# apache/auron

Measured on AMD Instinct MI355X. Metric: tpcds_suite_seconds, lower is better.
Workload: dtype decimal64/fp64

## Files before the change

auron_amd/config.py:

```python
from __future__ import annotations

import os
from dataclasses import dataclass
from typing import Any, Dict, Optional


@dataclass(frozen=True)
class ConfigOption:
    key: str
    default: Any
    typ: type
    doc: str = ""
    env: Optional[str] = None


_REGISTRY: Dict[str, ConfigOption] = {}


def _opt(key: str, default, typ, doc="", env=None) -> ConfigOption:
    o = ConfigOption(key, default, typ, doc, env)
    _REGISTRY[key] = o
    return o


# ... 55 lines not shown
                                    "below this many rows partial-agg "
                                    "skipping is never sampled")
SORT_LIMIT_TOPK = _opt("spark.auron.sort.topK.enable", True, bool,
                       "ORDER BY+LIMIT keeps only the top K rows per batch")
SORT_EXTERNAL_WIDE_KEYS = _opt("spark.auron.sort.external.wideKeys.enable",
                               True, bool,
                               "range-split external sort also for string and "
                               "decimal128 first keys (off: such sorts stay "
                               "monolithic and cannot spill)",
                               env="AURON_SORT_EXTERNAL_WIDE_KEYS")
EXCHANGE_SAMPLE_ROWS = _opt("spark.auron.rangePartition.sampleRows", 4096, int,
                            "per-rank sample size for range-partition bounds")
SCAN_CACHE_BYTES = _opt("spark.auron.scan.cache.maxBytes", 0, int,
                        "per-query decoded-scan cache budget; 0 = auto "
                        "(15% of HBM on GPU, 4 GB on CPU)",
                        env="AURON_SCAN_CACHE_BYTES")
STREAM_BYTES = _opt("spark.auron.stream.minInputBytes", -1, int,
                    "estimated agg-input bytes above which operators "
                    "stream instead of materializing; -1 = auto (8% of "
                    "HBM on GPU, 1 GB on CPU), 0 = always stream",
                    env="AURON_STREAM_BYTES")
SCAN_HBM_CACHE = _opt("spark.auron.scan.hbmStagedCache.maxBytes", 0, int,
                      "staged raw-page bytes kept device-resident across "
                      "reads; 0 = auto (30% of HBM)",
                      env="AURON_SCAN_HBM_CACHE")
HBM_CACHE_RESERVE = _opt("spark.auron.scan.hbmStagedCache.reserveFraction",
                         0.25, float,
                         "free-HBM fraction the staged-bytes cache must "
                         "never consume (evicts itself under pressure)")
SCAN_DELTA_NATIVE = _opt("spark.auron.scan.deltaNative.enable", True, bool,
                         "decode DELTA_BINARY_PACKED pages and "
                         "DELTA_LENGTH_BYTE_ARRAY / DELTA_BYTE_ARRAY string "
                         "pages with the k_pq_delta_* kernels from a "
                         "host-built miniblock index, DELTA_BYTE_ARRAY "
                         "strings rebuilt by k_pq_dba_bytes (off: "
                         "DELTA_BINARY_PACKED is expanded to PLAIN by one "
                         "host job per page and DELTA_LENGTH_BYTE_ARRAY and "
                         "DELTA_BYTE_ARRAY columns take the pyarrow host "
                         "read)",
                         env="AURON_SCAN_DELTA_NATIVE")
SCAN_PREFETCH = _opt("spark.auron.scan.streamPrefetch", 2, int,
                     "files decoded ahead of the consumer on the "
                     "streaming scan path")
SCAN_IO_THREADS = _opt("spark.auron.scan.ioThreads", 8, int,
                       "host page-read/staging thread-pool size",
                       env="AURON_SCAN_IO_THREADS")
STREAM_PEEK_FACTOR = _opt("spark.auron.stream.peekBatches", 8, int,
                          "batch-size multiples buffered before the "
                          "chunked agg commits to streaming")
STREAM_JOIN_PROBE = _opt("spark.auron.stream.joinProbe.enable", True, bool,
                         "probe build-right joins batch-by-batch on the "
                         "streaming path (GPU only)",
                         env="AURON_STREAM_JOIN_PROBE")
SPILL_DIR = _opt("spark.auron.spill.dir", "", str,
                 "directory for disk-tier spill files (empty = system tmp)",
                 env="AURON_SPILL_DIR")
MEM_BUDGET = _opt("spark.auron.memory.budgetBytes", 0, int,
                  "absolute memmgr budget override; 0 = memoryFraction "
                  "of device/host memory", env="AURON_MEM_BUDGET")


class AuronConf:
    def __init__(self, overrides: Optional[Dict[str, Any]] = None):
        self._values: Dict[str, Any] = {}
        if overrides:
            for k, v in overrides.items():
                self.set(k, v)

    def set(self, key: str, value) -> "AuronConf":
        if key not in _REGISTRY:
            raise KeyError(f"unknown config {key}; known: {sorted(_REGISTRY)}")
        self._values[key] = value
        return self

    def get(self, opt: ConfigOption):
        if opt.key in self._values:
            return self._values[opt.key]
        if opt.env and opt.env in os.environ:
            raw = os.environ[opt.env]
            if opt.typ is bool:
                return raw not in ("0", "false", "False")
            return opt.typ(raw)
        return opt.default

    @staticmethod
    def options() -> Dict[str, ConfigOption]:
        return dict(_REGISTRY)
```

auron_amd/engine/executor.py:

```python
from __future__ import annotations

import os
import time
from dataclasses import dataclass, field
from typing import Dict, List, Optional

import torch
import torch.distributed as dist

from .. import dtypes, ops
from ..column import Column, RecordBatch, adjacent_equal, compact_validity
from ..dtypes import DataType
from ..exchange import all_gather_batch, all_to_all
from ..exprs import AggFunc, Col
from ..plan import nodes as P
from ..config import AGG_STREAMING, BROADCAST_CACHE_BYTES, AuronConf
from .window import exec_window


@dataclass
class ExecContext:
    device: torch.device = torch.device("cpu")
    rank: int = 0
    world_size: int = 1
# ... 1744 lines not shown
                left = _concat(left_batches())
            else:
                lb = _concat(left_batches())
                left = _concat(all_gather_batch(lb, self.ctx.device, self.ctx.group))
                right = _concat(self.execute(node.right))
        else:
            right = _concat(self.execute(node.right))
            left = _concat(left_batches())
        if cache_entry is not None and cache_entry.get("batch") is None:
            cache_entry["batch"] = right
            self.ctx.broadcast_cache_bytes += sum(
                c.data.numel() * c.data.element_size() for c in right.columns)
        if not node.broadcast:
            from ..config import (SMJ_FALLBACK_ENABLE, SMJ_FALLBACK_ROWS,
                                  AuronConf)

            conf = AuronConf()
            build = right if node.build_side == "right" else left
            if (conf.get(SMJ_FALLBACK_ENABLE)
                    and build.num_rows > conf.get(SMJ_FALLBACK_ROWS)
                    and node.how in ("inner", "left", "right", "full",
                                     "semi", "anti", "existence")):
                smj = P.SortMergeJoin(P.MemoryScan([left]), P.MemoryScan([right]),
                                      node.left_keys, node.right_keys,
                                      how=node.how,
                                      existence_col=node.existence_col,
                                      residual=node.residual)
                return self._exec_SortMergeJoin(smj)
        lkeys = [k.eval(left) for k in node.left_keys]
        rkeys = [k.eval(right) for k in node.right_keys]
        lkeys, rkeys = _normalize_join_keys(lkeys, rkeys)
        how = node.how
        device = self.ctx.device

        table = None
        if cache_entry is not None and node.build_side == "right":
            sig = _expr_sig(node.right_keys)
            table = cache_entry["tables"].get(sig)
            if table is None:
                table = ops.join_build(rkeys)
                if table is not None:
                    cache_entry["tables"][sig] = table
                    self.ctx.broadcast_cache_bytes += table.nbytes

        if node.residual is not None:
            bi, pi, _ = ops.hash_join(rkeys, lkeys,
                                      emit_unmatched_probe=False,
                                      need_build_matched=False,
                                      table=table)
            return self._finish_join_pairs(left, right, pi, bi, how,
                                           node.residual, node.existence_col)

        if how in ("semi", "anti", "existence"):
            counts = ops.join_counts(rkeys, lkeys)
            if how == "semi":
                return [left.filter(counts > 0)]
            if how == "anti":
                return [left.filter(counts == 0)]
            exists = Column(dtypes.bool_, counts > 0)
            return [RecordBatch(left.names + [node.existence_col], left.columns + [exists])]

        preserved = {"inner": set(), "left": {"left"}, "right": {"right"},
                     "full": {"left", "right"}}[how]
        build_side = node.build_side
        probe_side = "left" if build_side == "right" else "right"
        build_keys, probe_keys = (rkeys, lkeys) if build_side == "right" else (lkeys, rkeys)
        bi, pi, bmatched = ops.hash_join(
            build_keys, probe_keys,
            emit_unmatched_probe=(probe_side in preserved),
            need_build_matched=(build_side in preserved),
            table=table if build_side == "right" else None,
        )
        if build_side in preserved and bmatched is not None:
            un = torch.nonzero(~bmatched, as_tuple=False).flatten()
            if un.numel():
                bi = torch.cat([bi, un])
                pi = torch.cat([pi, torch.full((un.numel(),), -1, dtype=torch.int64, device=bi.device)])
        li, ri = (pi, bi) if build_side == "right" else (bi, pi)
        out_left = left.gather(li, may_have_negative=True)
        out_right = right.gather(ri, may_have_negative=True)
        return [RecordBatch(out_left.names + out_right.names,
                            out_left.columns + out_right.columns)]

    def _finish_join_pairs(self, left: RecordBatch, right: RecordBatch,
                           li: torch.Tensor, ri: torch.Tensor, how: str,
                           residual, existence_col: str) -> List[RecordBatch]:
        device = self.ctx.device
        if residual is not None and li.numel():
            pair = RecordBatch(left.names + right.names,
                               left.gather(li).columns + right.gather(ri).columns)
            m = residual.eval(pair)
            keep = m.data
            if m.validity is not None:
                keep = keep & m.validity
            li, ri = li[keep], ri[keep]
        nl, nr = left.num_rows, right.num_rows
        if how in ("semi", "anti", "existence"):
            lmatched = torch.zeros(nl, dtype=torch.bool, device=device)
            if li.numel():
                lmatched[li] = True
            if how == "semi":
                return [left.filter(lmatched)]
            if how == "anti":
                return [left.filter(~lmatched)]
            return [RecordBatch(left.names + [existence_col],
                                left.columns + [Column(dtypes.bool_, lmatched)])]
        preserved = {"inner": set(), "left": {"left"}, "right": {"right"},
                     "full": {"left", "right"}}[how]
        if "left" in preserved:
            lm = torch.zeros(nl, dtype=torch.bool, device=device)
            if li.numel():
                lm[li] = True
# ... 53 lines not shown
```

auron_amd/exchange.py:

```python
from __future__ import annotations

from typing import List, Optional, Tuple

import torch
import torch.distributed as dist

from . import dtypes
from .column import Column, RecordBatch
from .dtypes import DataType

_ALIGN = 8


def _pad8(x: int) -> int:
    return (x + _ALIGN - 1) & ~(_ALIGN - 1)


def _byte_view(t: torch.Tensor) -> torch.Tensor:
    if t.numel() == 0:
        return torch.empty(0, dtype=torch.uint8, device=t.device)
    t = t.contiguous()
    if t.dtype == torch.bool:
        t = t.view(torch.uint8)
    t = t.view(torch.uint8) if t.dtype != torch.uint8 else t
# ... 109 lines not shown
        if b is None:
            metas.append(None)
            bufs.append(torch.zeros(0, dtype=torch.uint8, device=device))
        else:
            if schema is None:
                schema = _schema_of(b)
            m, buf = pack_batch(b, device)
            metas.append(m)
            bufs.append(buf)
    if schema is not None and all(m is not None for m in metas):
        ncols = len(schema)
        stride = 1 + 3 * ncols + 1
        comm_dev = device if dist.get_backend(group) == "nccl" else "cpu"
        sz = torch.full((world, stride), -1, dtype=torch.int64)
        for d, m in enumerate(metas):
            sz[d, 0] = m["nrows"]
            for i, cm in enumerate(m["cols"]):
                sz[d, 1 + 3 * i] = cm["data"]
                sz[d, 2 + 3 * i] = cm["val"]
                sz[d, 3 + 3 * i] = cm["off"]
            sz[d, -1] = bufs[d].numel()
        sz = sz.reshape(-1).to(comm_dev)
        outs = [torch.empty_like(sz) for _ in range(world)]
        dist.all_gather(outs, sz, group=group)
        rows = [o.cpu().reshape(world, stride)[rank] for o in outs]
        recv_metas = [_meta_from_sizes(schema, r) for r in rows]
        recv_sizes = [int(r[-1]) for r in rows]
    else:
        payload = (metas, [b.numel() for b in bufs])
        gathered: List[Optional[tuple]] = [None] * world
        dist.all_gather_object(gathered, payload, group=group)
        recv_metas = [gathered[s][0][rank] for s in range(world)]
        recv_sizes = [int(gathered[s][1][rank]) for s in range(world)]

    backend = dist.get_backend(group)
    out_batches: List[RecordBatch] = []
    if backend == "nccl":
        send_flat = torch.cat(bufs) if sum(b.numel() for b in bufs) else torch.zeros(0, dtype=torch.uint8, device=device)
        recv_total = sum(recv_sizes)
        recv_flat = torch.empty(recv_total, dtype=torch.uint8, device=device)
        dist.all_to_all_single(
            recv_flat, send_flat,
            output_split_sizes=recv_sizes,
            input_split_sizes=[b.numel() for b in bufs],
            group=group,
        )
        out_batches = _split_recv_flat(recv_flat, recv_sizes, recv_metas)
    else:
        recv_bufs: List[Optional[torch.Tensor]] = [None] * world
        recv_bufs[rank] = bufs[rank]
        for other in range(world):
            if other == rank:
                continue
            rb = torch.empty(recv_sizes[other], dtype=torch.uint8, device=device)
            if rank < other:
                if bufs[other].numel():
                    dist.send(bufs[other], dst=other, group=group)
                if rb.numel():
                    dist.recv(rb, src=other, group=group)
            else:
                if rb.numel():
                    dist.recv(rb, src=other, group=group)
                if bufs[other].numel():
                    dist.send(bufs[other], dst=other, group=group)
            recv_bufs[other] = rb
        for s in range(world):
            if recv_metas[s] is not None:
                out_batches.append(unpack_batch(recv_metas[s], recv_bufs[s]))
    return out_batches


def _split_recv_flat(recv_flat: torch.Tensor, recv_sizes, recv_metas):
    out = []
    pos = 0
    for s in range(len(recv_sizes)):
        nb = recv_sizes[s]
        if recv_metas[s] is not None:
            out.append(unpack_batch(recv_metas[s], recv_flat[pos:pos + nb]))
        pos += nb
    return out


def all_gather_batch(batch: Optional[RecordBatch], device, group=None) -> List[RecordBatch]:
    world = dist.get_world_size(group)
    if batch is not None:
        meta, buf = pack_batch(batch, device)
    else:
        meta, buf = None, torch.zeros(0, dtype=torch.uint8, device=device)
    gathered: List[Optional[tuple]] = [None] * world
    dist.all_gather_object(gathered, (meta, buf.numel()), group=group)
    all_meta = [g[0] for g in gathered]
    sizes = [g[1] for g in gathered]
    maxsz = max(sizes) if sizes else 0
    padded = torch.zeros(max(maxsz, 1), dtype=torch.uint8, device=device)
    if buf.numel():
        padded[:buf.numel()].copy_(buf)
    outs = [torch.empty(max(maxsz, 1), dtype=torch.uint8, device=device) for _ in range(world)]
    dist.all_gather(outs, padded, group=group)
    res = []
    for s in range(world):
        if all_meta[s] is not None:
            res.append(unpack_batch(all_meta[s], outs[s][:sizes[s]]))
    return res
```

auron_amd/native/__init__.py:

```python
from __future__ import annotations

import ctypes
import os
from typing import List, Optional, Tuple

import numpy as np
import torch

_LIB_NAME = "libauron_hip.so"
_here = os.path.dirname(os.path.abspath(__file__))
LIB_PATH = os.path.join(_here, _LIB_NAME)

_lib = None
_load_error: Optional[str] = None


class AuronNativeMissing(RuntimeError):
    pass


def _try_load():
    global _lib, _load_error
    if _lib is not None or _load_error is not None:
        return
    if not os.path.exists(LIB_PATH):
        _load_error = f"{LIB_PATH} not built (run python -m auron_amd.native.build)"
        return
    try:
        lib = ctypes.CDLL(LIB_PATH)
    except OSError as e:
        _load_error = str(e)
        return
    c = ctypes.c_void_p
    i32 = ctypes.c_int32
    i64 = ctypes.c_int64
    lib.au_abi_version.restype = ctypes.c_int
    lib.au_murmur3.argtypes = [c, ctypes.c_int, i64, i32, c, c]
    lib.au_group_ids.argtypes = [c, ctypes.c_int, i64, c, i64, c, c, c, c, c, c]
    lib.au_join_build.argtypes = [i64, c, i64, c, c, c]
    lib.au_join_count.argtypes = [c, c, ctypes.c_int, i64, c, i64, c, c, c, c]
    lib.au_join_fill.argtypes = [c, c, ctypes.c_int, i64, c, i64, c, c, c, c, c, c, ctypes.c_int, c]
    lib.au_pmod.argtypes = [c, i64, i32, c, c]
    lib.au_bytes_gather.argtypes = [c, c, c, c, i64, c]
    lib.au_multi_gather.argtypes = [c, i64, c, ctypes.c_int, c]
    lib.au_multi_gather.restype = ctypes.c_int
    lib.au_agg_scatter.argtypes = [c, i64, c, c, ctypes.c_int, ctypes.c_int,
                                   ctypes.c_int, c, c, i64, c]
    lib.au_agg_count.argtypes = [c, i64, c, c, c]
    lib.au_agg_multi.argtypes = [c, i64, c, ctypes.c_int, c]
    for f in ("au_agg_scatter", "au_agg_count", "au_agg_multi"):
        getattr(lib, f).restype = ctypes.c_int
    lib.au_pq_rle1.argtypes = [c, ctypes.c_int, c, c, c]
    lib.au_rle1_expand.argtypes = [c, i64, c, c, c]
    lib.au_rle1_expand.restype = ctypes.c_int
    lib.au_host_rle1_parse.argtypes = [c, i64, i64, i64, i64, c, i64]
    lib.au_host_rle1_parse.restype = i64
    lib.au_host_plainba_parse.argtypes = [c, i64, i64, c, c, i64]
    lib.au_host_plainba_parse.restype = i64
    lib.au_host_delta_unpack.argtypes = [c, i64, i64, i64, ctypes.c_int, c]
    lib.au_host_delta_unpack.restype = i64
    lib.au_host_delta_index.argtypes = [c, i64, i64, i64, i64, i64, i64, c, c,
                                        i64]
    lib.au_host_delta_index.restype = i64
    lib.au_pq_delta_sums.argtypes = [c, i64, c, c, c]
    lib.au_pq_delta_scan.argtypes = [c, i64, c]
    lib.au_pq_delta_emit.argtypes = [c, i64, c, i64, c, c, c, ctypes.c_int, c]
    for f in ("au_pq_delta_sums", "au_pq_delta_scan", "au_pq_delta_emit"):
        getattr(lib, f).restype = ctypes.c_int
    lib.au_host_dba_decode.argtypes = [c, i64, c, c, c, c, i64, c, i64]
    lib.au_host_dba_decode.restype = i64
    lib.au_pq_dba_tile.argtypes = []
    lib.au_pq_dba_tile.restype = i64
    lib.au_pq_dba_bytes.argtypes = [c, c, c, c, i64, i64, c, c, c]
    lib.au_pq_dba_bytes.restype = ctypes.c_int
    lib.au_pq_rle_idx.argtypes = [c, ctypes.c_int, c, c, c, c]
    lib.au_pq_scatter.argtypes = [c, ctypes.c_int, c, c, c, c, ctypes.c_int, i64, c]
    lib.au_pq_copy_plain.argtypes = [c, ctypes.c_int, c, c, ctypes.c_int, i64, c]
    for f in ("au_pq_rle1", "au_pq_rle_idx", "au_pq_scatter", "au_pq_copy_plain"):
        getattr(lib, f).restype = ctypes.c_int
    lib.au_expr_exec.argtypes = [c, ctypes.c_int, c, ctypes.c_int, c,
                                 ctypes.c_int, ctypes.c_int, i64, c]
    lib.au_expr_exec.restype = ctypes.c_int
    lib.au_part_hist.argtypes = [c, i64, i32, c, c]
    lib.au_part_scatter.argtypes = [c, i64, c, c, c, c]
    lib.au_range_bucket_str.argtypes = [c, c, i64, c, c, i32, ctypes.c_int, c, c]
    lib.au_range_bucket_i128.argtypes = [c, i64, c, i32, ctypes.c_int, c, c]
    for f in ("au_range_bucket_str", "au_range_bucket_i128"):
        getattr(lib, f).restype = ctypes.c_int
    f64 = ctypes.c_double
    lib.au_window_range_bounds_i64.argtypes = [c, c, c, i64, i64, i64,
                                               ctypes.c_int, c, c, c]
    lib.au_window_range_bounds_f64.argtypes = [c, c, c, i64, f64, f64,
                                               ctypes.c_int, c, c, c]
    lib.au_window_frame_minmax_i64.argtypes = [c, i64, c, i64, c, c, i64,
                                               ctypes.c_int, c, c]
    lib.au_window_frame_minmax_f64.argtypes = [c, i64, c, i64, c, c, i64,
                                               ctypes.c_int, c, c]
    lib.au_window_pyramid_size.argtypes = [i64]
    lib.au_window_pyramid_size.restype = i64
    lib.au_i128_scan_tile.argtypes = []
    lib.au_i128_scan_tile.restype = i64
    lib.au_prefix_sum_i128.argtypes = [c, c, i64, c, c, c]
    lib.au_window_frame_sum_i128.argtypes = [c, i64, c, c, i64, c, c]
    lib.au_window_frame_minmax_i128.argtypes = [c, i64, c, i64, c, c, i64,
                                                ctypes.c_int, c, c]
    for f in ("au_window_range_bounds_i64", "au_window_range_bounds_f64",
              "au_window_frame_minmax_i64", "au_window_frame_minmax_f64",
              "au_prefix_sum_i128", "au_window_frame_sum_i128",
              "au_window_frame_minmax_i128"):
        getattr(lib, f).restype = ctypes.c_int
    for f in ("au_murmur3", "au_group_ids", "au_join_build", "au_join_count",
              "au_join_fill", "au_pmod", "au_part_hist", "au_part_scatter"):
        getattr(lib, f).restype = ctypes.c_int
    _lib = lib


def available() -> bool:
    _try_load()
    return _lib is not None


def require():
    _try_load()
    if _lib is None:
        raise AuronNativeMissing(
            f"auron native HIP library unavailable: {_load_error}. "
            "Build it with `python -m auron_amd.native.build`."
        )
    return _lib


def lib():
    return require()


def host_lib():
    return require()


_DESC_DTYPE = np.dtype(
    [("data", "<u8"), ("offsets", "<u8"), ("validity", "<u8"),
     ("dtype", "<i4"), ("scale", "<i4")]
)
assert _DESC_DTYPE.itemsize == 32


def pack_descs(cols, device) -> Tuple[torch.Tensor, list]:
    n = len(cols)
    arr = np.zeros(n, dtype=_DESC_DTYPE)
    keep = []
    for i, col in enumerate(cols):
        data = col.data
        if not data.is_contiguous():
            data = data.contiguous()
        keep.append(data)
        arr[i]["data"] = data.data_ptr()
        if col.offsets is not None:
            off = col.offsets.contiguous()
            keep.append(off)
            arr[i]["offsets"] = off.data_ptr()
        if col.validity is not None:
            v = col.validity.contiguous()
            keep.append(v)
            arr[i]["validity"] = v.data_ptr()
        arr[i]["dtype"] = col.dtype.code
        arr[i]["scale"] = col.dtype.scale
    from ..pinned import to_device

    dev = to_device(arr.view(np.uint8).reshape(-1), device)
    keep.append(dev)
    return dev, keep


def stream_ptr(device) -> ctypes.c_void_p:
    return ctypes.c_void_p(torch.cuda.current_stream(device).cuda_stream)


def check(rc: int, what: str):
    if rc != 0:
        raise RuntimeError(f"native kernel {what} failed with hipError {rc}")
    if os.environ.get("AURON_SYNC_NATIVE", "0") == "1":
        torch.cuda.synchronize()
```

auron_amd/native/csrc/kernels.hip:

```cpp

#include <hip/hip_runtime.h>
#include <stdint.h>

#define AU_EXPORT extern "C" __attribute__((visibility("default")))

enum AuDType : int32_t {
  AU_BOOL = 0,
  AU_INT8 = 1,
  AU_INT16 = 2,
  AU_INT32 = 3,
  AU_INT64 = 4,
  AU_FLOAT32 = 5,
  AU_FLOAT64 = 6,
  AU_DATE32 = 7,
  AU_STRING = 8,
  AU_DECIMAL64 = 9,
  AU_LIST = 10,
  AU_TIMESTAMP = 11,
};

struct AuColDesc {
  const void* data;
  const int64_t* offsets;
  const uint8_t* validity;
// ... 279 lines not shown
    if (!join_row_has_null(pcols, ncols, i)) {
      int32_t j = heads[((uint32_t)phashes[i]) & cap_mask];
      while (j != -1) {
        if (keys_equal(bcols, j, pcols, i, ncols) &&
            !join_row_has_null(bcols, ncols, j)) {
          build_out[o] = j;
          probe_out[o] = i;
          if (build_matched) build_matched[j] = 1;
          o++;
        }
        j = next[j];
      }
    }
    if (emit_unmatched_probe && o == start) {
      build_out[o] = -1;
      probe_out[o] = i;
    }
  }
}

AU_EXPORT int au_join_build(int64_t n, int32_t* heads, int64_t cap,
                            int32_t* next, const int32_t* hashes, void* stream) {
  if (n == 0) return 0;
  hipLaunchKernelGGL(k_join_build, dim3(au_grid(n, 256)), dim3(256), 0,
                     (hipStream_t)stream, n, heads, (uint32_t)(cap - 1), next,
                     hashes);
  return (int)hipGetLastError();
}

AU_EXPORT int au_join_count(const void* bcols, const void* pcols, int ncols,
                            int64_t n_probe, const int32_t* heads, int64_t cap,
                            const int32_t* next, const int32_t* phashes,
                            int32_t* counts, void* stream) {
  if (n_probe == 0) return 0;
  hipLaunchKernelGGL(k_join_count, dim3(au_grid(n_probe, 256)), dim3(256), 0,
                     (hipStream_t)stream, (const AuColDesc*)bcols,
                     (const AuColDesc*)pcols, ncols, n_probe, heads,
                     (uint32_t)(cap - 1), next, phashes, counts);
  return (int)hipGetLastError();
}

AU_EXPORT int au_join_fill(const void* bcols, const void* pcols, int ncols,
                           int64_t n_probe, const int32_t* heads, int64_t cap,
                           const int32_t* next, const int32_t* phashes,
                           const int64_t* offsets, int64_t* build_out,
                           int64_t* probe_out, uint8_t* build_matched,
                           int emit_unmatched_probe, void* stream) {
  if (n_probe == 0) return 0;
  hipLaunchKernelGGL(k_join_fill, dim3(au_grid(n_probe, 256)), dim3(256), 0,
                     (hipStream_t)stream, (const AuColDesc*)bcols,
                     (const AuColDesc*)pcols, ncols, n_probe, heads,
                     (uint32_t)(cap - 1), next, phashes, offsets, build_out,
                     probe_out, build_matched, emit_unmatched_probe);
  return (int)hipGetLastError();
}

__global__ void k_pmod(const int32_t* hashes, int64_t n, int32_t nparts,
                       int32_t* part_ids) {
  for (int64_t i = (int64_t)blockIdx.x * blockDim.x + threadIdx.x; i < n;
       i += (int64_t)gridDim.x * blockDim.x) {
    int32_t m = hashes[i] % nparts;
    part_ids[i] = m < 0 ? m + nparts : m;
  }
}

AU_EXPORT int au_pmod(const int32_t* hashes, int64_t n, int32_t nparts,
                      int32_t* part_ids, void* stream) {
  if (n == 0) return 0;
  hipLaunchKernelGGL(k_pmod, dim3(au_grid(n, 256)), dim3(256), 0,
                     (hipStream_t)stream, hashes, n, nparts, part_ids);
  return (int)hipGetLastError();
}

__global__ void k_part_hist(const int32_t* part_ids, int64_t n, int32_t nparts,
                            int32_t* counts) {
  for (int64_t i = (int64_t)blockIdx.x * blockDim.x + threadIdx.x; i < n;
       i += (int64_t)gridDim.x * blockDim.x) {
    atomicAdd(&counts[part_ids[i]], 1);
  }
}

__global__ void k_part_scatter(const int32_t* part_ids, int64_t n,
                               const int64_t* base, int32_t* cursors,
                               int64_t* order) {
  for (int64_t i = (int64_t)blockIdx.x * blockDim.x + threadIdx.x; i < n;
       i += (int64_t)gridDim.x * blockDim.x) {
    int32_t p = part_ids[i];
    int64_t slot = base[p] + atomicAdd(&cursors[p], 1);
    order[slot] = i;
  }
}

AU_EXPORT int au_part_hist(const int32_t* part_ids, int64_t n, int32_t nparts,
                           int32_t* counts, void* stream) {
  if (n == 0) return 0;
  hipLaunchKernelGGL(k_part_hist, dim3(au_grid(n, 256)), dim3(256), 0,
                     (hipStream_t)stream, part_ids, n, nparts, counts);
  return (int)hipGetLastError();
}

AU_EXPORT int au_part_scatter(const int32_t* part_ids, int64_t n,
                              const int64_t* base, int32_t* cursors,
                              int64_t* order, void* stream) {
  if (n == 0) return 0;
  hipLaunchKernelGGL(k_part_scatter, dim3(au_grid(n, 256)), dim3(256), 0,
                     (hipStream_t)stream, part_ids, n, base, cursors, order);
// ... 92 lines not shown
```

auron_amd/ops.py:

```python
from __future__ import annotations

import os
from typing import List, Optional, Tuple

import torch

from . import dtypes, native
from .column import Column

SPARK_SEED = 42
_M32 = 0xFFFFFFFF


def _use_native(device: torch.device) -> bool:
    if device.type != "cuda":
        return False
    if os.environ.get("AURON_FORCE_REF", "0") == "1":
        return False
    if os.environ.get("AURON_REQUIRE_NATIVE", "1") == "0" and not native.available():
        return False
    native.require()
    return True


# ... 182 lines not shown
    matched = [False] * n_build
    bi, pi = [], []
    for i, k in enumerate(pkeys):
        rows = [] if any(v is None for v in k) else table.get(k, [])
        if rows:
            for j in rows:
                bi.append(j)
                pi.append(i)
                matched[j] = True
        elif emit_unmatched_probe:
            bi.append(-1)
            pi.append(i)
    device = probe_cols[0].device
    bm = torch.tensor(matched, dtype=torch.bool, device=device) if need_build_matched else None
    return (torch.tensor(bi, dtype=torch.int64, device=device),
            torch.tensor(pi, dtype=torch.int64, device=device), bm)



class JoinTable:

    __slots__ = ("heads", "nxt", "cap", "bhash", "n_build")

    def __init__(self, heads, nxt, cap, bhash, n_build):
        self.heads = heads
        self.nxt = nxt
        self.cap = cap
        self.bhash = bhash
        self.n_build = n_build

    @property
    def nbytes(self):
        return (self.heads.numel() + self.nxt.numel()) * 4 + self.bhash.numel() * 8


def join_build(build_cols: List[Column]) -> Optional["JoinTable"]:
    device = build_cols[0].device
    if not _use_native(device):
        return None
    lib = native.lib()
    sp = native.stream_ptr(device)
    n_build = len(build_cols[0])
    bhash = murmur3(build_cols)
    cap = _next_pow2(2 * max(n_build, 1))
    heads = torch.full((cap,), -1, dtype=torch.int32, device=device)
    nxt = torch.empty(max(n_build, 1), dtype=torch.int32, device=device)
    if n_build:
        rc = lib.au_join_build(n_build, heads.data_ptr(), cap, nxt.data_ptr(),
                               bhash.data_ptr(), sp)
        native.check(rc, "au_join_build")
    return JoinTable(heads, nxt, cap, bhash, n_build)


def hash_join(build_cols: List[Column], probe_cols: List[Column],
              emit_unmatched_probe: bool = False,
              need_build_matched: bool = False,
              table: Optional["JoinTable"] = None):
    device = probe_cols[0].device
    n_probe = len(probe_cols[0])
    n_build = len(build_cols[0])
    if not _use_native(device):
        return hash_join_ref(build_cols, probe_cols, emit_unmatched_probe, need_build_matched)
    lib = native.lib()
    sp = native.stream_ptr(device)
    if table is None:
        table = join_build(build_cols)
    heads, nxt, cap, bhash = table.heads, table.nxt, table.cap, table.bhash
    phash = murmur3(probe_cols)
    bdescs, bkeep = native.pack_descs(build_cols, device)
    pdescs, pkeep = native.pack_descs(probe_cols, device)
    counts = torch.zeros(n_probe, dtype=torch.int32, device=device)
    rc = lib.au_join_count(bdescs.data_ptr(), pdescs.data_ptr(), len(build_cols),
                           n_probe, heads.data_ptr(), cap, nxt.data_ptr(),
                           phash.data_ptr(), counts.data_ptr(), sp)
    native.check(rc, "au_join_count")
    eff = counts.to(torch.int64)
    if emit_unmatched_probe:
        eff = eff.clamp(min=1)
    offsets = torch.zeros(n_probe + 1, dtype=torch.int64, device=device)
    torch.cumsum(eff, 0, out=offsets[1:])
    total = int(offsets[-1].item())
    build_idx = torch.empty(max(total, 1), dtype=torch.int64, device=device)
    probe_idx = torch.empty(max(total, 1), dtype=torch.int64, device=device)
    bm = torch.zeros(n_build, dtype=torch.uint8, device=device) if need_build_matched else None
    rc = lib.au_join_fill(bdescs.data_ptr(), pdescs.data_ptr(), len(build_cols),
                          n_probe, heads.data_ptr(), cap, nxt.data_ptr(),
                          phash.data_ptr(), offsets.data_ptr(),
                          build_idx.data_ptr(), probe_idx.data_ptr(),
                          bm.data_ptr() if bm is not None else None,
                          1 if emit_unmatched_probe else 0, sp)
    native.check(rc, "au_join_fill")
    del bkeep, pkeep
    return build_idx[:total], probe_idx[:total], (bm.bool() if bm is not None else None)


def join_counts(build_cols: List[Column], probe_cols: List[Column]) -> torch.Tensor:
    device = probe_cols[0].device
    n_probe = len(probe_cols[0])
    n_build = len(build_cols[0])
    if not _use_native(device):
        bi, pi, _ = hash_join_ref(build_cols, probe_cols, False, False)
        counts = torch.zeros(n_probe, dtype=torch.int32)
        if pi.numel():
            counts.scatter_add_(0, pi, torch.ones(pi.numel(), dtype=torch.int32))
        return counts
    lib = native.lib()
    sp = native.stream_ptr(device)
    bhash = murmur3(build_cols)
    phash = murmur3(probe_cols)
    cap = _next_pow2(2 * max(n_build, 1))
    heads = torch.full((cap,), -1, dtype=torch.int32, device=device)
    nxt = torch.empty(max(n_build, 1), dtype=torch.int32, device=device)
    bdescs, bkeep = native.pack_descs(build_cols, device)
    pdescs, pkeep = native.pack_descs(probe_cols, device)
    if n_build:
        rc = lib.au_join_build(n_build, heads.data_ptr(), cap, nxt.data_ptr(),
                               bhash.data_ptr(), sp)
        native.check(rc, "au_join_build")
    counts = torch.zeros(n_probe, dtype=torch.int32, device=device)
    rc = lib.au_join_count(bdescs.data_ptr(), pdescs.data_ptr(), len(build_cols),
                           n_probe, heads.data_ptr(), cap, nxt.data_ptr(),
                           phash.data_ptr(), counts.data_ptr(), sp)
    native.check(rc, "au_join_count")
    del bkeep, pkeep
    return counts


def string_sort_ranks(c: Column) -> torch.Tensor:
    gids, reps = group_ids([c])
    rep_vals = c.gather(reps).to_pylist()
    order = sorted(range(len(rep_vals)),
                   key=lambda i: (rep_vals[i] is None, rep_vals[i] or ""))
    rank = [0] * len(rep_vals)
    for r, i in enumerate(order):
        rank[i] = r
    rank_t = torch.tensor(rank, dtype=torch.int64, device=c.device)
    return rank_t[gids]


_MIN64 = -(1 << 63)


def _bytes_cmp_sign(a_data, a_start, a_len, b_data, b_start, b_len,
                    chunk: int = 64) -> torch.Tensor:
    n = a_start.numel()
    device = a_start.device
# ... 639 lines not shown
```

Baseline: 3.251.

## Add fused hash-join probe kernels with in-kernel hashing and tile offsets

Adds fused HIP kernels for join probe count/fill and semi/anti existence. They compute the probe hash inside the kernel, walk the chain once, record the first match, and build per-tile offsets in place of a full-length cumsum. Key descriptors are passed by value, which avoids a host-to-device descriptor copy, and there are specialized single int64/int32 key paths. Semi/anti joins now reuse the cached broadcast table through join_exists. Separately, the exchange send/recv and all_gather now stage buffers through the CPU for non-NCCL backends, which may add host copies.

```diff
diff --git a/auron_amd/config.py b/auron_amd/config.py
--- a/auron_amd/config.py
+++ b/auron_amd/config.py
@@ -131,6 +131,15 @@
                          "probe build-right joins batch-by-batch on the "
                          "streaming path (GPU only)",
                          env="AURON_STREAM_JOIN_PROBE")
+JOIN_FUSED_PROBE = _opt("spark.auron.join.fusedProbe.enable", True, bool,
+                        "probe hash joins with the fused kernels "
+                        "(k_join_probe_count / k_join_probe_fill / "
+                        "k_join_exists: probe hash computed in-kernel, one "
+                        "chain walk, per-tile offsets, key descriptors passed "
+                        "by value) for up to 8 key columns (off: murmur3 + "
+                        "k_join_count + torch scan + k_join_fill, and "
+                        "join_counts for semi/anti/existence joins)",
+                        env="AURON_JOIN_FUSED_PROBE")
 SPILL_DIR = _opt("spark.auron.spill.dir", "", str,
                  "directory for disk-tier spill files (empty = system tmp)",
                  env="AURON_SPILL_DIR")
diff --git a/auron_amd/engine/executor.py b/auron_amd/engine/executor.py
--- a/auron_amd/engine/executor.py
+++ b/auron_amd/engine/executor.py
@@ -1820,12 +1820,12 @@
                                            node.residual, node.existence_col)
 
         if how in ("semi", "anti", "existence"):
-            counts = ops.join_counts(rkeys, lkeys)
+            matched = ops.join_exists(rkeys, lkeys, table=table)
             if how == "semi":
-                return [left.filter(counts > 0)]
+                return [left.filter(matched)]
             if how == "anti":
-                return [left.filter(counts == 0)]
-            exists = Column(dtypes.bool_, counts > 0)
+                return [left.filter(~matched)]
+            exists = Column(dtypes.bool_, matched)
             return [RecordBatch(left.names + [node.existence_col], left.columns + [exists])]
 
         preserved = {"inner": set(), "left": {"left"}, "right": {"right"},
diff --git a/auron_amd/exchange.py b/auron_amd/exchange.py
--- a/auron_amd/exchange.py
+++ b/auron_amd/exchange.py
@@ -185,18 +185,19 @@
         for other in range(world):
             if other == rank:
                 continue
-            rb = torch.empty(recv_sizes[other], dtype=torch.uint8, device=device)
+            sb = bufs[other].cpu()
+            rb = torch.empty(recv_sizes[other], dtype=torch.uint8)
             if rank < other:
-                if bufs[other].numel():
-                    dist.send(bufs[other], dst=other, group=group)
+                if sb.numel():
+                    dist.send(sb, dst=other, group=group)
                 if rb.numel():
                     dist.recv(rb, src=other, group=group)
             else:
                 if rb.numel():
                     dist.recv(rb, src=other, group=group)
-                if bufs[other].numel():
-                    dist.send(bufs[other], dst=other, group=group)
-            recv_bufs[other] = rb
+                if sb.numel():
+                    dist.send(sb, dst=other, group=group)
+            recv_bufs[other] = rb.to(device)
         for s in range(world):
             if recv_metas[s] is not None:
                 out_batches.append(unpack_batch(recv_metas[s], recv_bufs[s]))
@@ -225,13 +226,14 @@
     all_meta = [g[0] for g in gathered]
     sizes = [g[1] for g in gathered]
     maxsz = max(sizes) if sizes else 0
-    padded = torch.zeros(max(maxsz, 1), dtype=torch.uint8, device=device)
+    comm_dev = device if dist.get_backend(group) == "nccl" else "cpu"
+    padded = torch.zeros(max(maxsz, 1), dtype=torch.uint8, device=comm_dev)
     if buf.numel():
         padded[:buf.numel()].copy_(buf)
-    outs = [torch.empty(max(maxsz, 1), dtype=torch.uint8, device=device) for _ in range(world)]
+    outs = [torch.empty(max(maxsz, 1), dtype=torch.uint8, device=comm_dev) for _ in range(world)]
     dist.all_gather(outs, padded, group=group)
     res = []
     for s in range(world):
         if all_meta[s] is not None:
-            res.append(unpack_batch(all_meta[s], outs[s][:sizes[s]]))
+            res.append(unpack_batch(all_meta[s], outs[s][:sizes[s]].to(device)))
     return res
diff --git a/auron_amd/native/__init__.py b/auron_amd/native/__init__.py
--- a/auron_amd/native/__init__.py
+++ b/auron_amd/native/__init__.py
@@ -40,6 +40,17 @@
     lib.au_join_build.argtypes = [i64, c, i64, c, c, c]
     lib.au_join_count.argtypes = [c, c, ctypes.c_int, i64, c, i64, c, c, c, c]
     lib.au_join_fill.argtypes = [c, c, ctypes.c_int, i64, c, i64, c, c, c, c, c, c, ctypes.c_int, c]
+    lib.au_join_probe_tile.argtypes = []
+    lib.au_join_probe_tile.restype = i64
+    lib.au_join_probe_max_keys.argtypes = []
+    lib.au_join_probe_max_keys.restype = ctypes.c_int
+    lib.au_join_probe_count.argtypes = [c, ctypes.c_int, i64, c, i64, c, i32,
+                                        ctypes.c_int, c, c, c, c, c]
+    lib.au_join_probe_fill.argtypes = [c, ctypes.c_int, i64, c, c, c, c,
+                                       ctypes.c_int, c, c, c]
+    lib.au_join_exists.argtypes = [c, ctypes.c_int, i64, c, i64, c, i32, c, c]
+    for f in ("au_join_probe_count", "au_join_probe_fill", "au_join_exists"):
+        getattr(lib, f).restype = ctypes.c_int
     lib.au_pmod.argtypes = [c, i64, i32, c, c]
     lib.au_bytes_gather.argtypes = [c, c, c, c, i64, c]
     lib.au_multi_gather.argtypes = [c, i64, c, ctypes.c_int, c]
@@ -145,7 +156,7 @@
 assert _DESC_DTYPE.itemsize == 32
 
 
-def pack_descs(cols, device) -> Tuple[torch.Tensor, list]:
+def pack_descs_host(cols) -> Tuple[np.ndarray, list]:
     n = len(cols)
     arr = np.zeros(n, dtype=_DESC_DTYPE)
     keep = []
@@ -165,6 +176,11 @@
             arr[i]["validity"] = v.data_ptr()
         arr[i]["dtype"] = col.dtype.code
         arr[i]["scale"] = col.dtype.scale
+    return arr, keep
+
+
+def pack_descs(cols, device) -> Tuple[torch.Tensor, list]:
+    arr, keep = pack_descs_host(cols)
     from ..pinned import to_device
 
     dev = to_device(arr.view(np.uint8).reshape(-1), device)
diff --git a/auron_amd/native/csrc/kernels.hip b/auron_amd/native/csrc/kernels.hip
--- a/auron_amd/native/csrc/kernels.hip
+++ b/auron_amd/native/csrc/kernels.hip
@@ -355,6 +355,279 @@
                      (const AuColDesc*)pcols, ncols, n_probe, heads,
                      (uint32_t)(cap - 1), next, phashes, offsets, build_out,
                      probe_out, build_matched, emit_unmatched_probe);
+  return (int)hipGetLastError();
+}
+
+#define JP_MAX_KEYS 8
+#define JP_BLOCK 256
+#define JP_SLABS 4
+#define JP_TILE (JP_BLOCK * JP_SLABS)
+
+struct JpKeys {
+  AuColDesc build[JP_MAX_KEYS];
+  AuColDesc probe[JP_MAX_KEYS];
+};
+
+template <int MODE>
+__device__ __forceinline__ bool jp_probe_key(const JpKeys& k, int ncols,
+                                             int64_t i, int64_t* pkey) {
+  if (MODE == 0) return !join_row_has_null(k.probe, ncols, i);
+  const uint8_t* v = k.probe[0].validity;
+  if (v != nullptr && v[i] == 0) return false;
+  if (MODE == 1) *pkey = ((const int64_t*)k.probe[0].data)[i];
+  else *pkey = ((const int32_t*)k.probe[0].data)[i];
+  return true;
+}
+
+template <int MODE>
+__device__ __forceinline__ uint32_t jp_hash(const JpKeys& k, int ncols,
+                                            int64_t i, int64_t pkey,
+                                            uint32_t seed) {
+  if (MODE == 1) return hash_long((uint64_t)pkey, seed);
+  if (MODE == 2) return hash_int((uint32_t)(int32_t)pkey, seed);
+  uint32_t h = seed;
+  for (int c = 0; c < ncols; c++) h = hash_one(k.probe[c], i, h);
+  return h;
+}
+
+template <int MODE>
+__device__ __forceinline__ bool jp_match(const JpKeys& k, int ncols, int32_t j,
+                                         int64_t i, int64_t pkey) {
+  if (MODE == 0)
+    return keys_equal(k.build, j, k.probe, i, ncols) &&
+           !join_row_has_null(k.build, ncols, j);
+  const uint8_t* v = k.build[0].validity;
+  if (MODE == 1) {
+    if (((const int64_t*)k.build[0].data)[j] != pkey) return false;
+  } else {
+    if (((const int32_t*)k.build[0].data)[j] != (int32_t)pkey) return false;
+  }
+  return v == nullptr || v[j] != 0;
+}
+
+template <int MODE>
+__global__ void __launch_bounds__(JP_BLOCK) k_join_probe_count(
+    JpKeys k, int ncols, int64_t n_probe, int64_t n_tiles,
+    const int32_t* __restrict__ heads, uint32_t cap_mask,
+    const int32_t* __restrict__ next, uint32_t seed, int emit_unmatched_probe,
+    int32_t* __restrict__ counts, int32_t* __restrict__ first,
+    int64_t* __restrict__ tile_sums, uint8_t* build_matched) {
+  __shared__ int64_t wsum[JP_BLOCK / 64];
+  const int tid = threadIdx.x;
+  for (int64_t t = blockIdx.x; t < n_tiles; t += gridDim.x) {
+    const int64_t base = t * JP_TILE;
+    int32_t j0[JP_SLABS];
+    int64_t pk[JP_SLABS];
+#pragma unroll
+    for (int s = 0; s < JP_SLABS; s++) {
+      const int64_t i = base + s * JP_BLOCK + tid;
+      j0[s] = -1;
+      pk[s] = 0;
+      if (i < n_probe && jp_probe_key<MODE>(k, ncols, i, &pk[s]))
+        j0[s] = heads[jp_hash<MODE>(k, ncols, i, pk[s], seed) & cap_mask];
+    }
+    int64_t acc = 0;
+#pragma unroll
+    for (int s = 0; s < JP_SLABS; s++) {
+      const int64_t i = base + s * JP_BLOCK + tid;
+      if (i >= n_probe) continue;
+      int32_t cnt = 0, f = -1;
+      for (int32_t j = j0[s]; j != -1; j = next[j]) {
+        if (jp_match<MODE>(k, ncols, j, i, pk[s])) {
+          if (cnt == 0) f = j;
+          cnt++;
+          if (build_matched) build_matched[j] = 1;
+        }
+      }
+      counts[i] = cnt;
+      first[i] = f;
+      acc += (emit_unmatched_probe && cnt == 0) ? 1 : cnt;
+    }
+    for (int d = 32; d > 0; d >>= 1) acc += __shfl_down(acc, d, 64);
+    if ((tid & 63) == 0) wsum[tid >> 6] = acc;
+    __syncthreads();
+    if (tid == 0) {
+      int64_t sum = 0;
+      for (int w = 0; w < JP_BLOCK / 64; w++) sum += wsum[w];
+      tile_sums[t] = sum;
+    }
+    __syncthreads();
+  }
+}
+
+template <int MODE>
+__global__ void __launch_bounds__(JP_BLOCK) k_join_probe_fill(
+    JpKeys k, int ncols, int64_t n_probe, int64_t n_tiles,
+    const int32_t* __restrict__ next, const int32_t* __restrict__ counts,
+    const int32_t* __restrict__ first, const int64_t* __restrict__ tile_ends,
+    int emit_unmatched_probe, int64_t* __restrict__ build_out,
+    int64_t* __restrict__ probe_out) {
+  __shared__ int64_t wtot[2][JP_BLOCK / 64];
+  const int tid = threadIdx.x;
+  const int lane = tid & 63, wave = tid >> 6;
+  for (int64_t t = blockIdx.x; t < n_tiles; t += gridDim.x) {
+    const int64_t base = t * JP_TILE;
+    int64_t running = t == 0 ? 0 : tile_ends[t - 1];
+    for (int s = 0; s < JP_SLABS; s++) {
+      const int64_t i = base + s * JP_BLOCK + tid;
+      const bool in = i < n_probe;
+      const int32_t cnt = in ? counts[i] : 0;
+      const int64_t eff = !in ? 0 : (emit_unmatched_probe && cnt == 0) ? 1 : cnt;
+      int64_t incl = eff;
+      for (int d = 1; d < 64; d <<= 1) {
+        int64_t up = __shfl_up(incl, d, 64);
+        if (lane >= d) incl += up;
+      }
+      if (lane == 63) wtot[s & 1][wave] = incl;
+      __syncthreads();
+      int64_t before = 0, total = 0;
+      for (int w = 0; w < JP_BLOCK / 64; w++) {
+        const int64_t x = wtot[s & 1][w];
+        if (w < wave) before += x;
+        total += x;
+      }
+      int64_t o = running + before + incl - eff;
+      running += total;
+      if (!in) continue;
+      if (cnt == 0) {
+        if (emit_unmatched_probe) {
+          build_out[o] = -1;
+          probe_out[o] = i;
+        }
+      } else if (cnt == 1) {
+        build_out[o] = first[i];
+        probe_out[o] = i;
+      } else {
+        int64_t pkey = 0;
+        jp_probe_key<MODE>(k, ncols, i, &pkey);
+        int32_t left = cnt;
+        for (int32_t j = first[i]; j != -1 && left > 0; j = next[j]) {
+          if (jp_match<MODE>(k, ncols, j, i, pkey)) {
+            build_out[o] = j;
+            probe_out[o] = i;
+            o++;
+            left--;
+          }
+        }
+      }
+    }
+  }
+}
+
+template <int MODE>
+__global__ void __launch_bounds__(JP_BLOCK) k_join_exists(
+    JpKeys k, int ncols, int64_t n_probe, const int32_t* __restrict__ heads,
+    uint32_t cap_mask, const int32_t* __restrict__ next, uint32_t seed,
+    uint8_t* __restrict__ out) {
+  for (int64_t i = (int64_t)blockIdx.x * blockDim.x + threadIdx.x; i < n_probe;
+       i += (int64_t)gridDim.x * blockDim.x) {
+    uint8_t found = 0;
+    int64_t pkey = 0;
+    if (jp_probe_key<MODE>(k, ncols, i, &pkey)) {
+      int32_t j = heads[jp_hash<MODE>(k, ncols, i, pkey, seed) & cap_mask];
+      while (j != -1) {
+        if (jp_match<MODE>(k, ncols, j, i, pkey)) {
+          found = 1;
+          break;
+        }
+        j = next[j];
+      }
+    }
+    out[i] = found;
+  }
+}
+
+static inline bool jp_int64_family(int32_t d) {
+  return d == AU_INT64 || d == AU_DECIMAL64 || d == AU_TIMESTAMP;
+}
+static inline bool jp_int32_family(int32_t d) {
+  return d == AU_INT32 || d == AU_DATE32;
+}
+
+static int jp_pack(const void* host_descs, int ncols, JpKeys* k) {
+  const AuColDesc* d = (const AuColDesc*)host_descs;
+  for (int c = 0; c < ncols; c++) {
+    k->build[c] = d[c];
+    k->probe[c] = d[ncols + c];
+  }
+  if (ncols == 1) {
+    if (jp_int64_family(d[0].dtype) && jp_int64_family(d[1].dtype)) return 1;
+    if (jp_int32_family(d[0].dtype) && jp_int32_family(d[1].dtype)) return 2;
+  }
+  return 0;
+}
+
+static inline int jp_grid(int64_t n_tiles) {
+  return (int)(n_tiles > 2048 ? 2048 : n_tiles);
+}
+
+AU_EXPORT int64_t au_join_probe_tile() { return JP_TILE; }
+AU_EXPORT int au_join_probe_max_keys() { return JP_MAX_KEYS; }
+
+AU_EXPORT int au_join_probe_count(const void* host_descs, int ncols,
+                                  int64_t n_probe, const int32_t* heads,
+                                  int64_t cap, const int32_t* next,
+                                  int32_t seed, int emit_unmatched_probe,
+                                  int32_t* counts, int32_t* first,
+                                  int64_t* tile_sums, uint8_t* build_matched,
+                                  void* stream) {
+  if (n_probe == 0) return 0;
+  if (ncols < 1 || ncols > JP_MAX_KEYS) return 1002;
+  JpKeys k{};
+  const int mode = jp_pack(host_descs, ncols, &k);
+  const int64_t n_tiles = (n_probe + JP_TILE - 1) / JP_TILE;
+#define JP_LAUNCH_COUNT(M)                                                     \
+  hipLaunchKernelGGL(k_join_probe_count<M>, dim3(jp_grid(n_tiles)),            \
+                     dim3(JP_BLOCK), 0, (hipStream_t)stream, k, ncols, n_probe, \
+                     n_tiles, heads, (uint32_t)(cap - 1), next, (uint32_t)seed, \
+                     emit_unmatched_probe, counts, first, tile_sums,           \
+                     build_matched)
+  if (mode == 1) JP_LAUNCH_COUNT(1);
+  else if (mode == 2) JP_LAUNCH_COUNT(2);
+  else JP_LAUNCH_COUNT(0);
+#undef JP_LAUNCH_COUNT
+  return (int)hipGetLastError();
+}
+
+AU_EXPORT int au_join_probe_fill(const void* host_descs, int ncols,
+                                 int64_t n_probe, const int32_t* next,
+                                 const int32_t* counts, const int32_t* first,
+                                 const int64_t* tile_ends,
+                                 int emit_unmatched_probe, int64_t* build_out,
+                                 int64_t* probe_out, void* stream) {
+  if (n_probe == 0) return 0;
+  if (ncols < 1 || ncols > JP_MAX_KEYS) return 1002;
+  JpKeys k{};
+  const int mode = jp_pack(host_descs, ncols, &k);
+  const int64_t n_tiles = (n_probe + JP_TILE - 1) / JP_TILE;
+#define JP_LAUNCH_FILL(M)                                                      \
+  hipLaunchKernelGGL(k_join_probe_fill<M>, dim3(jp_grid(n_tiles)),             \
+                     dim3(JP_BLOCK), 0, (hipStream_t)stream, k, ncols, n_probe, \
+                     n_tiles, next, counts, first, tile_ends,                  \
+                     emit_unmatched_probe, build_out, probe_out)
+  if (mode == 1) JP_LAUNCH_FILL(1);
+  else if (mode == 2) JP_LAUNCH_FILL(2);
+  else JP_LAUNCH_FILL(0);
+#undef JP_LAUNCH_FILL
+  return (int)hipGetLastError();
+}
+
+AU_EXPORT int au_join_exists(const void* host_descs, int ncols, int64_t n_probe,
+                             const int32_t* heads, int64_t cap,
+                             const int32_t* next, int32_t seed, uint8_t* out,
+                             void* stream) {
+  if (n_probe == 0) return 0;
+  if (ncols < 1 || ncols > JP_MAX_KEYS) return 1002;
+  JpKeys k{};
+  const int mode = jp_pack(host_descs, ncols, &k);
+#define JP_LAUNCH_EXISTS(M)                                                    \
+  hipLaunchKernelGGL(k_join_exists<M>, dim3(au_grid(n_probe, JP_BLOCK)),       \
+                     dim3(JP_BLOCK), 0, (hipStream_t)stream, k, ncols, n_probe, \
+                     heads, (uint32_t)(cap - 1), next, (uint32_t)seed, out)
+  if (mode == 1) JP_LAUNCH_EXISTS(1);
+  else if (mode == 2) JP_LAUNCH_EXISTS(2);
+  else JP_LAUNCH_EXISTS(0);
+#undef JP_LAUNCH_EXISTS
   return (int)hipGetLastError();
 }
 
diff --git a/auron_amd/ops.py b/auron_amd/ops.py
--- a/auron_amd/ops.py
+++ b/auron_amd/ops.py
@@ -258,6 +258,27 @@
     return JoinTable(heads, nxt, cap, bhash, n_build)
 
 
+JOIN_PROBE_MAX_KEYS = 8
+
+
+def _fused_probe_enabled() -> bool:
+    from .config import JOIN_FUSED_PROBE, AuronConf
+
+    return bool(AuronConf().get(JOIN_FUSED_PROBE))
+
+
+def join_probe_tile() -> int:
+    return int(native.lib().au_join_probe_tile())
+
+
+def _join_key_descs(build_cols, probe_cols):
+    import numpy as np
+
+    barr, bkeep = native.pack_descs_host(build_cols)
+    parr, pkeep = native.pack_descs_host(probe_cols)
+    return np.concatenate([barr, parr]), (bkeep, pkeep)
+
+
 def hash_join(build_cols: List[Column], probe_cols: List[Column],
               emit_unmatched_probe: bool = False,
               need_build_matched: bool = False,
@@ -267,10 +288,62 @@
     n_build = len(build_cols[0])
     if not _use_native(device):
         return hash_join_ref(build_cols, probe_cols, emit_unmatched_probe, need_build_matched)
-    lib = native.lib()
-    sp = native.stream_ptr(device)
     if table is None:
         table = join_build(build_cols)
+    if len(build_cols) <= JOIN_PROBE_MAX_KEYS and _fused_probe_enabled():
+        return _hash_join_fused(build_cols, probe_cols, emit_unmatched_probe,
+                                need_build_matched, table)
+    return _hash_join_legacy(build_cols, probe_cols, emit_unmatched_probe,
+                             need_build_matched, table)
+
+
+def _hash_join_fused(build_cols, probe_cols, emit_unmatched_probe,
+                     need_build_matched, table):
+    device = probe_cols[0].device
+    n_probe = len(probe_cols[0])
+    n_build = len(build_cols[0])
+    lib = native.lib()
+    sp = native.stream_ptr(device)
+    bm = torch.zeros(n_build, dtype=torch.uint8, device=device) if need_build_matched else None
+    if n_probe == 0:
+        empty = torch.empty(0, dtype=torch.int64, device=device)
+        return empty, empty.clone(), (bm.bool() if bm is not None else None)
+    ncols = len(build_cols)
+    descs, keep = _join_key_descs(build_cols, probe_cols)
+    tile = join_probe_tile()
+    n_tiles = (n_probe + tile - 1) // tile
+    counts = torch.empty(n_probe, dtype=torch.int32, device=device)
+    first = torch.empty(n_probe, dtype=torch.int32, device=device)
+    tile_sums = torch.empty(n_tiles, dtype=torch.int64, device=device)
+    emit = 1 if emit_unmatched_probe else 0
+    rc = lib.au_join_probe_count(descs.ctypes.data, ncols, n_probe,
+                                 table.heads.data_ptr(), table.cap,
+                                 table.nxt.data_ptr(), SPARK_SEED, emit,
+                                 counts.data_ptr(), first.data_ptr(),
+                                 tile_sums.data_ptr(),
+                                 bm.data_ptr() if bm is not None and n_build else None,
+                                 sp)
+    native.check(rc, "au_join_probe_count")
+    tile_ends = torch.cumsum(tile_sums, 0)
+    total = int(tile_ends[-1].item())
+    build_idx = torch.empty(max(total, 1), dtype=torch.int64, device=device)
+    probe_idx = torch.empty(max(total, 1), dtype=torch.int64, device=device)
+    rc = lib.au_join_probe_fill(descs.ctypes.data, ncols, n_probe,
+                                table.nxt.data_ptr(), counts.data_ptr(),
+                                first.data_ptr(), tile_ends.data_ptr(), emit,
+                                build_idx.data_ptr(), probe_idx.data_ptr(), sp)
+    native.check(rc, "au_join_probe_fill")
+    del keep
+    return build_idx[:total], probe_idx[:total], (bm.bool() if bm is not None else None)
+
+
+def _hash_join_legacy(build_cols, probe_cols, emit_unmatched_probe,
+                      need_build_matched, table):
+    device = probe_cols[0].device
+    n_probe = len(probe_cols[0])
+    n_build = len(build_cols[0])
+    lib = native.lib()
+    sp = native.stream_ptr(device)
     heads, nxt, cap, bhash = table.heads, table.nxt, table.cap, table.bhash
     phash = murmur3(probe_cols)
     bdescs, bkeep = native.pack_descs(build_cols, device)
@@ -298,6 +371,33 @@
     native.check(rc, "au_join_fill")
     del bkeep, pkeep
     return build_idx[:total], probe_idx[:total], (bm.bool() if bm is not None else None)
+
+
+def join_exists(build_cols: List[Column], probe_cols: List[Column],
+                table: Optional["JoinTable"] = None) -> torch.Tensor:
+    device = probe_cols[0].device
+    n_probe = len(probe_cols[0])
+    if not _use_native(device):
+        _, pi, _ = hash_join_ref(build_cols, probe_cols, False, False)
+        out = torch.zeros(n_probe, dtype=torch.bool, device=device)
+        if pi.numel():
+            out[pi] = True
+        return out
+    if len(build_cols) > JOIN_PROBE_MAX_KEYS or not _fused_probe_enabled():
+        return join_counts(build_cols, probe_cols) > 0
+    if table is None:
+        table = join_build(build_cols)
+    out = torch.empty(n_probe, dtype=torch.bool, device=device)
+    if n_probe:
+        descs, keep = _join_key_descs(build_cols, probe_cols)
+        rc = native.lib().au_join_exists(descs.ctypes.data, len(build_cols),
+                                         n_probe, table.heads.data_ptr(),
+                                         table.cap, table.nxt.data_ptr(),
+                                         SPARK_SEED, out.data_ptr(),
+                                         native.stream_ptr(device))
+        native.check(rc, "au_join_exists")
+        del keep
+    return out
 
 
 def join_counts(build_cols: List[Column], probe_cols: List[Column]) -> torch.Tensor:
diff --git a/profiles/measure_join_probe.py b/profiles/measure_join_probe.py
--- /dev/null
+++ b/profiles/measure_join_probe.py
@@ -0,0 +1,114 @@
+import argparse
+import json
+import os
+import statistics
+import sys
+
+import torch
+
+sys.path.insert(0, os.path.join(os.path.dirname(os.path.abspath(__file__)), ".."))
+from auron_amd import dtypes, native, ops
+from auron_amd.column import Column
+
+DEV = "cuda:0"
+
+
+def _int_col(t):
+    return Column(dtypes.int64, t.to(DEV), None, None)
+
+
+def _str_col(ids):
+    import numpy as np
+
+    a = np.char.zfill(ids.numpy().astype(str), 11)
+    raw = np.char.add("k", a).astype("S12")
+    data = torch.from_numpy(np.frombuffer(raw.tobytes(), dtype=np.uint8).copy())
+    offs = torch.arange(0, 12 * (len(ids) + 1), 12, dtype=torch.int64)
+    return Column(dtypes.string, data.to(DEV), None, offs.to(DEV))
+
+
+def _timed(fn, switch_env, warm, reps):
+    out, ts = {}, {"0": [], "1": []}
+    for s in ("0", "1"):
+        os.environ[switch_env] = s
+        for _ in range(warm):
+            out[s] = fn()
+    torch.cuda.synchronize()
+    for _ in range(reps):
+        for s in ("0", "1"):
+            os.environ[switch_env] = s
+            e0 = torch.cuda.Event(enable_timing=True)
+            e1 = torch.cuda.Event(enable_timing=True)
+            e0.record()
+            out[s] = fn()
+            e1.record()
+            torch.cuda.synchronize()
+            ts[s].append(e0.elapsed_time(e1))
+    os.environ.pop(switch_env, None)
+
+    def stat(v):
+        return {"median": round(statistics.median(v), 4), "min": round(min(v), 4),
+                "max": round(max(v), 4)}
+
+    return out["0"], out["1"], stat(ts["0"]), stat(ts["1"])
+
+
+def _same(a, b):
+    a = a if isinstance(a, tuple) else (a,)
+    b = b if isinstance(b, tuple) else (b,)
+    return all((x is None and y is None) or torch.equal(x, y) for x, y in zip(a, b))
+
+
+def main():
+    ap = argparse.ArgumentParser()
+    ap.add_argument("--rows", type=int, default=16_000_000)
+    ap.add_argument("--reps", type=int, default=20)
+    args = ap.parse_args()
+    assert torch.cuda.is_available(), "needs a GPU"
+    native.require()
+    n = args.rows
+    g = torch.Generator().manual_seed(0)
+    env = "AURON_JOIN_FUSED_PROBE"
+
+    def report(name, n_probe, n_build, res):
+        off, on, t_off, t_on = res
+        first = on[0] if isinstance(on, tuple) else on
+        print(json.dumps({"case": name, "probe_rows": n_probe, "build_rows": n_build,
+                          "out_rows": int(first.numel()) if isinstance(on, tuple)
+                          else int(first.sum().item()),
+                          "same_result": _same(off, on),
+                          "legacy_ms": t_off, "fused_ms": t_on,
+                          "speedup_median": round(t_off["median"] / t_on["median"], 3)}),
+              flush=True)
+
+    def join_case(name, build_ids, probe_ids, emit=False, as_str=False):
+        mk = _str_col if as_str else _int_col
+        b, p = [mk(build_ids)], [mk(probe_ids)]
+        table = ops.join_build(b)
+        res = _timed(lambda: ops.hash_join(b, p, emit, False, table=table),
+                     env, 3, args.reps)
+        report(name, len(probe_ids), len(build_ids), res)
+
+    join_case("73k unique build, ~20% match", torch.randperm(73_000, generator=g),
+              torch.randint(0, 365_000, (n,), generator=g))
+    join_case("500k unique build, all match", torch.randperm(500_000, generator=g),
+              torch.randint(0, 500_000, (n,), generator=g))
+    dup_build = torch.randperm(2_000_000, generator=g) // 4
+    join_case("2M build, 4 rows per key, all match", dup_build,
+              torch.randint(0, 500_000, (n,), generator=g))
+    join_case("left join, 500k unique build, ~50% match",
+              torch.randperm(500_000, generator=g),
+              torch.randint(0, 1_000_000, (n,), generator=g), emit=True)
+    join_case("string key, 100k build, 4M probe", torch.randperm(100_000, generator=g),
+              torch.randint(0, 120_000, (min(n, 4_000_000),), generator=g), as_str=True)
+
+    b, p = [_int_col(dup_build)], [_int_col(torch.randint(0, 600_000, (n,), generator=g))]
+    table = ops.join_build(b)
+    for name, tb in (("exists vs counts, cached table", table),
+                     ("exists vs counts, no cached table", None)):
+        res = _timed(lambda: ops.join_exists(b, p, table=tb), env, 3, args.reps)
+        report(name, n, len(dup_build), res)
+
+
+if __name__ == "__main__":
+    main()
```

New measurement: 3.057 (median of 6 runs). 1.06x faster.
